# XiandaGuo/OpenStereo

Measured on AMD Instinct MI355X. Metric: stereo-pairs/s at 540x960 D=192 (GwcNet fwd), higher is better.
Workload: dtype f32 via f16x3 split-MFMA (hi/lo fp16 operands, f32 accumulate; HBM tensors f32); 1 GPU; GwcNet-gc inference, SceneFlow-shaped 540x960 padded to 544x960, D=192, G=40 + 12ch concat (BASELINE configs[1]); weights=deterministic synthetic (sharpened), random-init architecture, sub_batch_streams=3, parallelism=independent pairs x1, precision=f16x3, launch=hipGraph replay

## Files before the change

include/openstereo_amd.h:

```cpp
#ifndef OPENSTEREO_AMD_H
#define OPENSTEREO_AMD_H

#include <stddef.h>

#ifdef __cplusplus
extern "C" {
#endif

#define OSA_ABI_VERSION 16
#define OSA_META_FLOATS 128

enum { OSA_NCDHW = 0, OSA_NDHWC = 1 };
enum { OSA_ACT_NONE = 0, OSA_ACT_RELU = 1, OSA_ACT_LEAKY = 2, OSA_ACT_RELU6 = 3, OSA_ACT_SIGMOID = 4, OSA_ACT_TANH = 5 };
enum { OSA_GATE_RAW = 16 };
#define OSA_GATE_CHANNELS(n) ((int)((unsigned)(n) << 16))
enum { OSA_IN_SPLIT = 32, OSA_OUT_SPLIT = 64, OSA_RES_SPLIT = 128, OSA_REDIR_SPLIT = 256 };
enum { OSA_RES_AFTER_ACT = 512 };

int         osa_abi_version(void);
const char* osa_last_error(void);
const char* osa_target_arch(void);

int osa_build_volume_f32(const float* left_gwc, const float* right_gwc, int C, int num_groups,
                         const float* left_cat, const float* right_cat, int Cc,
                         float* vol, int layout, int vol_channels, int c_off,
                         int B, int H, int W, int maxdisp, int mask_left_concat,
                         float* vol_meta, void* stream);

int osa_build_volume_nhwc_f32(const float* left_gwc, const float* right_gwc, int C, int num_groups, int gwc_stride,
                              const float* left_cat, const float* right_cat, int Cc, int cat_stride,
                              float* vol, int vol_channels, int c_off,
                              int B, int H, int W, int maxdisp, int mask_left_concat, float* vol_meta, void* stream);
int osa_cat_fms_f32(const float* reference_fm, const float* target_fm, float* out, const int* disp_index,
                    int B, int C, int H, int W, int n_samples, void* stream);
int osa_pair_volume_f32(const float* left, const float* right, float* out,
                        int B, int C, int groups, int H, int W, int planes, int mode, void* stream);

int osa_corr_volume_f32(const float* left, const float* right, float* vol,
                        int B, int C, int H, int W, int maxdisp, void* stream);

int osa_ncdhw_to_ndhwc_f32(const float* x, float* y, int B, int C, long long S,
                           int yCs, int c_off, void* stream);
// ... 333 lines not shown

enum { OSA_IN_F16 = 32, OSA_OUT_F16 = 64, OSA_RES_F16 = 128 };
int osa_conv3d_pack_f16(const float* w_ref, float* w_packed, int Ci, int Co, int kd, int kh, int kw, void* stream);
int osa_deconv3d_pack_f16(const float* w_ref, float* w_packed, int Ci, int Co, int k, int pad, void* stream);
int osa_deconv2d_pack_f16(const float* w_ref, float* w_packed, int Ci, int Co, int k, int pad, void* stream);
int osa_conv3d_ndhwc_f16(const void* x, const float* w_packed, const float* scale, const float* shift, const void* residual, void* y,
                         int B, int Di, int Hi, int Wi, int Ci, int xCs, int Co, int yCs, int rCs, int kd, int kh, int kw, int stride,
                         int pad_d, int pad_h, int pad_w, int dil_d, int dil_h, int dil_w, const float* gate_logits, int gCs,
                         int act, float slope, void* stream);
int osa_deconv3d_ndhwc_f16(const void* x, const float* w_packed, const float* scale, const float* shift, const void* residual, void* y,
                           int B, int Di, int Hi, int Wi, int Ci, int xCs, int Co, int yCs, int rCs, int k, int pad, int opad,
                           const float* gate_logits, int gCs, int act, float slope, void* stream);
int osa_deconv2d_nhwc_f16(const void* x, const float* w_packed, const float* scale, const float* shift, const void* residual, void* y,
                          int B, int Hi, int Wi, int Ci, int xCs, int Co, int yCs, int rCs, int k, int pad, int opad,
                          const float* gate_logits, int gCs, int act, float slope, void* stream);

size_t osa_channel_sums_workspace_bytes(long long P, int C);
int osa_channel_sums(const void* dy, int dy_f16, int dy_cs, const void* x, int x_f16, int x_cs, const float* x_shift,
                     const float* dx_scale, void* dx, int dx_cs, long long P, int C,
                     float* out, float* workspace, size_t workspace_bytes, void* stream);
int osa_channel_sums_multi(const void* const* dys, int n_items, int dy_f16, int dy_cs, long long P, int C,
                           float* out, float* workspace, size_t workspace_bytes, void* stream);
int osa_channel_affine(const void* u, int u_f16, int u_cs, const void* v, int v_f16, int v_cs,
                       const float* a, const float* b, const float* c0, void* out, int out_cs,
                       long long P, int C, int relu, void* stream);

size_t osa_instnorm_workspace_floats(int B, long long HW, int C);
int osa_instnorm_nhwc_f32(const float* x, float* y, int B, long long HW, int C, int xCs, int yCs, float eps, int act, float slope,
                          float* workspace, float* y_meta, void* stream);

long long osa_conv3d_march_launches(void);

long long osa_conv3d_march_s2_launches(void);

int osa_deconv_walk(int enable);
int osa_deconv_walk_segment_planes(int planes);
long long osa_deconv3d_walk_launches(void);

int osa_conv_b_ring_mask(int mask);
long long osa_conv_b_ring_launches(void);

int osa_volume_walk_step(int step);
long long osa_volume_walk_launches(void);

int osa_build_volume_nhwc_split_eligible(const float* left_cat, const float* right_cat, const float* vol, int C, int num_groups,
                                         int gwc_stride, int Cc, int cat_stride, int vol_channels, int c_off, int W, int maxdisp);
int osa_build_volume_nhwc_split_f16x3(const float* left_gwc, const float* right_gwc, int C, int num_groups, int gwc_stride,
                                      const float* left_cat, const float* right_cat, int Cc, int cat_stride,
                                      float* vol, int vol_channels, int c_off,
                                      int B, int H, int W, int maxdisp, int mask_left_concat,
                                      const float* gwc_meta, const float* cat_meta, float* vol_meta, void* stream);

#ifdef __cplusplus
}
#endif
#endif
```

openstereo_amd/_lib.py:

```python
from __future__ import annotations

import ctypes as C
import os
import threading

_HERE = os.path.dirname(os.path.abspath(__file__))
LIB_PATH = os.environ.get("OSA_LIB_PATH") or os.path.join(_HERE, "lib", "libopenstereo_amd.so")

_lock = threading.Lock()
_lib = None

c_fp = C.c_void_p
c_i = C.c_int
c_f = C.c_float
c_st = C.c_void_p
c_ll = C.c_longlong


class F16x3Ranges(C.Structure):
    _fields_ = [("x_meta", C.c_void_p), ("residual_meta", C.c_void_p), ("redir_meta", C.c_void_p),
                ("y_meta", C.c_void_p), ("bound_coef", C.c_void_p), ("redir_bound_coef", C.c_void_p), ("weight_scale", C.c_void_p)]


c_rng = C.POINTER(F16x3Ranges)
# ... 44 lines not shown
    "osa_deconv2d_nhwc_f16x3": (c_i, [c_fp] * 6 + [c_i] * 11 + [c_fp, c_i, c_i, c_f, c_f, c_rng, c_st]),
    "osa_dwconv2d_pack_f32": (c_i, [c_fp, c_fp, c_i, c_i, c_i, c_st]),
    "osa_dwconv2d_nhwc_f32": (c_i, [c_fp] * 6 + [c_i] * 15 + [c_fp, c_st]),
    "osa_dwconv2d_nhwc_f16io": (c_i, [c_fp, c_i, c_fp, c_fp, c_fp, c_fp, c_i] + [c_i] * 11 + [c_i, c_fp, c_st]),
    "osa_gru_combine_f32": (c_i, [c_fp, c_fp, c_fp, c_fp, c_ll, c_i, c_i, c_i, c_i, c_i, c_fp, c_st]),
    "osa_gru_gates_rz_fwd": (c_i, [c_ref, c_fp, c_fp, c_ref, c_ref, c_ref, c_ref, c_ref, c_ll, c_i, c_st]),
    "osa_gru_gates_rz_bwd": (c_i, [c_ref, c_fp, c_fp, c_ref, c_ref, c_ref, c_ref, c_ref, c_ref, c_ref, c_ll, c_i, c_st]),
    "osa_gru_gates_q_fwd": (c_i, [c_ref, c_ref, c_fp, c_ref, c_ref, c_ref, c_ll, c_i, c_st]),
    "osa_gru_gates_q_bwd": (c_i, [c_ref, c_ref, c_fp, c_ref, c_ref, c_ref, c_ref, c_ref, c_ref, c_ll, c_i, c_st]),
    "osa_disp_update_f32": (c_i, [c_fp, c_fp, c_i, c_fp, c_fp, c_i, c_ll, c_fp, c_fp, c_st]),
    "osa_conv3d_pack_ex_auto": (c_i, [c_fp, c_fp, c_i, c_i, c_i, c_i, c_i, c_i, c_i, c_fp, c_fp, c_st]),
    **dict.fromkeys(("osa_deconv3d_pack_f16x3_auto", "osa_deconv2d_pack_f16x3_auto"), (c_i, [c_fp, c_fp, c_i, c_i, c_i, c_i, c_fp, c_fp, c_st])),
    "osa_cat_fms_f32": (c_i, [c_fp, c_fp, c_fp, c_fp, c_i, c_i, c_i, c_i, c_i, c_st]),
    "osa_pool2x_nhwc_f32": (c_i, [c_fp, c_fp, c_i, c_i, c_i, c_i, c_i, c_i, c_fp, c_fp, c_st]),
    "osa_resize_bilinear_nhwc_f32": (c_i, [c_fp, c_fp, c_i, c_i, c_i, c_i, c_i, c_i, c_i, c_i, c_fp, c_fp, c_st]),
    "osa_context_upsample_logits_f32": (c_i, [c_fp, c_fp, c_i, C.POINTER(c_ll), c_fp, c_i, c_i, c_i, c_i, c_f, c_st]),
    "osa_context_upsample_logits_bwd_f32": (c_i, [c_fp, c_fp, c_i, C.POINTER(c_ll), c_fp, c_fp, c_fp, C.POINTER(c_ll), c_fp, c_i, c_i, c_i, c_i, c_f, c_st]),
    "osa_context_upsample_f32": (c_i, [c_fp, c_fp, c_fp, c_i, c_i, c_i, c_i, c_i, c_f, c_st]),
    "osa_geo_rows_f32": (c_i, [c_fp, c_fp, c_i, c_i, c_i, c_i, c_i, c_i, c_st]),
    "osa_avgpool_rows_f32": (c_i, [c_fp, c_fp, c_ll, c_i, c_st]),
    **dict.fromkeys(("osa_geo_lookup_f32", "osa_geo_lookup_bwd_acc_f32", "osa_geo_lookup_bwd_f32"), (c_i, _LEVELS + [c_fp, c_fp, c_fp, c_i, c_i, c_i, c_i, c_i, c_st])),
    "osa_geo_lookup_nhwc_f32": (c_i, _LEVELS + [c_fp, c_fp, c_fp, c_i, c_i, c_i, c_i, c_i, c_i, c_st]),
    **dict.fromkeys(("osa_geo_lookup_mr_f32", "osa_geo_lookup_mr_bwd_acc_f32"), (c_i, _LEVELS + [c_fp, c_i, c_fp, c_i, c_fp, c_fp, c_fp, c_fp, c_fp, c_fp, c_i, c_i, c_i, c_i, c_i, c_st])),
    "osa_geo_lookup_mr_nhwc_f32": (c_i, _LEVELS + [c_fp, c_i, c_fp, c_i, c_fp, c_fp, c_fp, c_fp, c_fp, c_fp, c_i, c_i, c_i, c_i, c_i, c_i, c_i, c_i, c_i, c_st]),
    "osa_preprocess_pair_f32": (c_i, [c_fp, c_fp, c_i, c_i, c_i, c_i, c_i, C.POINTER(c_f), C.POINTER(c_f), c_fp, c_i, c_st]),
    "osa_instnorm_workspace_floats": (C.c_size_t, [c_i, c_ll, c_i]),
    "osa_instnorm_nhwc_f32": (c_i, [c_fp, c_fp, c_i, c_ll, c_i, c_i, c_i, c_f, c_i, c_f, c_fp, c_fp, c_st]),
    "osa_conv3d_wgrad_ws_multi": (c_i, [c_i, c_fp, c_fp, c_i, c_fp] + [c_i] * 22 + [c_fp, c_fp, c_i, c_i, c_fp, C.c_size_t, c_st]),
    "osa_channel_sums_workspace_bytes": (C.c_size_t, [c_ll, c_i]),
    "osa_channel_affine": (c_i, [c_fp, c_i, c_i, c_fp, c_i, c_i, c_fp, c_fp, c_fp, c_fp, c_i, c_ll, c_i, c_i, c_st]),
    "osa_channel_sums_multi": (c_i, [c_fp, c_i, c_i, c_i, c_ll, c_i, c_fp, c_fp, C.c_size_t, c_st]),
    "osa_channel_sums": (c_i, [c_fp, c_i, c_i, c_fp, c_i, c_i, c_fp, c_fp, c_fp, c_i, c_ll, c_i, c_fp, c_fp, C.c_size_t, c_st]),
    **dict.fromkeys(("osa_conv3d_march_launches", "osa_conv3d_march_s2_launches", "osa_deconv3d_walk_launches", "osa_conv_b_ring_launches", "osa_volume_walk_launches"), (c_ll, [])),
    **dict.fromkeys(("osa_deconv_walk", "osa_deconv_walk_segment_planes", "osa_conv_b_ring_mask", "osa_volume_walk_step"), (c_i, [c_i])),
    "osa_build_volume_nhwc_split_eligible": (c_i, [c_fp, c_fp, c_fp, c_i, c_i, c_i, c_i, c_i, c_i, c_i, c_i, c_i]),
    "osa_build_volume_nhwc_split_f16x3": (c_i, [c_fp, c_fp, c_i, c_i, c_i, c_fp, c_fp, c_i, c_i, c_fp] + [c_i] * 7 + [c_fp, c_fp, c_fp, c_st]),
    "osa_upsample_softargmin_f32": (c_i, [c_fp, c_fp, c_i, c_i, c_i, c_i, c_i, c_i, c_i, c_i, c_st]),
    **dict.fromkeys(("osa_softargmin_var_f32", "osa_softmax_softargmin_var_bwd_f32"), (c_i, [c_fp, c_fp, c_fp, c_fp, c_i, c_i, c_i, c_i, c_st])),
    "osa_softargmin_var_bwd_f32": (c_i, [c_fp, c_fp, c_fp, c_fp, c_fp, c_fp, c_i, c_i, c_i, c_i, c_st]),
    "osa_upsample_softargmin_var_bwd_ws_f32": (c_i, [c_fp, c_fp, c_fp, c_fp, c_i, c_i, c_i, c_i, c_i, c_i, c_i, c_i, c_fp, C.c_size_t, c_st]),
    "osa_mr_volume_f32": (c_i, [c_fp] * 7 + [c_i] * 12 + [c_st]),
    "osa_mr_volume_bwd_ws_f32": (c_i, [c_fp] * 3 + [c_i] + [c_fp] * 8 + [c_i] * 11 + [c_fp, C.c_size_t, c_st]),
    **dict.fromkeys(("osa_mv2_block3d_packed_floats", "osa_mv2_block2d_packed_floats"), (C.c_size_t, [c_i] * 3)),
    **dict.fromkeys(("osa_mv2_block3d_pack_f32", "osa_mv2_block2d_pack_f32"), (c_i, [c_fp] * 10 + [c_i] * 3 + [c_st])),
    "osa_mv2_block3d_f32": (c_i, [c_fp] * 3 + [c_i] * 9 + [c_st]),
    **dict.fromkeys(("osa_mv2_block2d_f32", "osa_disparity_attention_f32"), (c_i, [c_fp] * 4 + [c_i] * 9 + [c_st])),
    "osa_disparity_attention_pack_f32": (c_i, [c_fp] * 8 + [c_i] * 4 + [c_st]),
    "osa_interlaced_volume_pack_f32": (c_i, [c_fp] * 13 + [c_i] * 4 + [c_st]),
    "osa_interlaced_volume_f32": (c_i, [c_fp] * 4 + [c_i] * 8 + [c_st]),
}


class EngineError(RuntimeError):
    pass


def load():
    global _lib
    if _lib is not None:
        return _lib
    with _lock:
        if _lib is not None:
            return _lib
        if not os.path.exists(LIB_PATH):
            raise EngineError(f"{LIB_PATH} is missing: build it with `python -m openstereo_amd.build` (hipcc, gfx950). There is no CPU fallback.")
        lib = C.CDLL(LIB_PATH)
        for name, (res, args) in SIGNATURES.items():
# ... 46 lines not shown
```

openstereo_amd/csrc/conv3d.hip:

```cpp
#include "conv_kernel.h"
#include "conv_inst.h"

namespace osa {

struct KernelCfg {
    const char* name;
    int M, N;
    int TD, TH, TW, threads;
    int ks;
    int table, idx;
};

static const KernelCfg g_cfgs[] = {
#define OSA_CFG_X(RING, MT, NT, WM, WN, TH, TW)                                                                  \
    { #MT "x" #NT "_" #WM "x" #WN "_" #TH "x" #TW, WM * MT * 32, WN * NT * 32, WM * MT * 32 / (TH * TW), TH, TW, WM * WN * 64, 0, 0, -1 },
#define OSA_KS_X(MT, NT, WM, WN, TH, TW, KS)
#include "conv_cfgs.def"
#undef OSA_CFG_X
#undef OSA_KS_X
};
constexpr int N_CFGS = sizeof(g_cfgs) / sizeof(g_cfgs[0]);

static const KernelCfg g_ks_cfgs[] = {
#define OSA_CFG_X(RING, MT, NT, WM, WN, TH, TW)
// ... 132 lines not shown
    static Key cache[64]; static int used = 0;
    for (int i = 0; i < used; ++i) if (cache[i].f == (const void*)fn && cache[i].l == lds) return cache[i].n;
    int n = 0;
    if (hipOccupancyMaxActiveBlocksPerMultiprocessor(&n, (const void*)fn, threads, lds) != hipSuccess) { (void)hipGetLastError(); n = 1; }
    if (used < 64) cache[used++] = Key{(const void*)fn, lds, n};
    return n;
}

static void set_stagger(ConvArgs& a, const KernelCfg& k, void (*fn)(const ConvArgs), size_t lds, long long nwg, bool deconv, int prec) {
    a.stag_ticks = 0; a.stag_n = 0; a.stag_cus = 256;
    const int mode = exp_int("OSA_STAG", 0);
    if (!mode) return;
    const int waves = k.threads / 64;
    int slots = resident_workgroups(fn, k.threads, lds);
    { const int o = exp_int("OSA_STAG_K", 0); if (o) slots = o; }
    if (slots < 2 || nwg < (long long)2 * slots * 256) return;
    const double mfma_per_wave = (double)a.nchunks * a.T * ((double)k.M * k.N / 1024.0 / waves) * (prec == PREC_F16X3 ? 3.0 : 8.0);
    const double tap_us = mfma_per_wave * (prec == PREC_F16X3 ? 32.0 : 64.0) / 2000.0;
    const double bytes = (double)a.LD * a.LH * a.LW * 64.0 * a.nchunks + (double)k.M * (deconv ? 8 : 1) * k.N * 4.0 * (a.res || a.rx ? 2 : 1);
    const double mem_us = bytes / (4.0e6 / 256.0);
    double step_us = tap_us > mem_us ? tap_us : mem_us;
    if ((tap_us + mem_us) / slots > step_us) step_us = (tap_us + mem_us) / slots;
    { const int o = exp_int("OSA_STAG_PCT", 100); step_us *= o / 100.0; }
    { const int o = exp_int("OSA_STAG_US10", 0); if (o) step_us = o / 10.0; }
    a.stag_ticks = (int)(step_us * 100.0 + 0.5);
    a.stag_n = slots * 256; a.stag_cus = 256;
    if (exp_int("OSA_STAG_PRINT", 0)) fprintf(stderr, "[stagger] %s slots %d tap %.2f us mem %.2f us step %.2f us\n", k.name, slots, tap_us, mem_us, step_us);
}

int launch_conv_march(ConvArgs& a, hipStream_t st, const char* what);
int launch_conv_march_s2(ConvArgs& a, hipStream_t st, const char* what);
int launch_conv_deconv_walk(ConvArgs& a, hipStream_t st, const char* what);
void wgrad_set_multi_tile(int on);
void march_s2_set_waves(int w);

static int g_b_ring_mask = (1 << 1) | (1 << 2) | (1 << 3) | (1 << 4) | (1 << 13) | (1 << 29) | (1 << 27);
static long long g_b_ring_launches = 0;
static int g_b_ring_mask_value() { return g_b_ring_mask; }

static int plan_conv(ConvArgs& a, int stride, int prec, const char* what, const KernelCfg* forced, const KernelCfg*& kp) {
    int ci = forced ? 0 : pick_cfg(a, stride, prec);
    if (!forced && brick_bytes(a, g_cfgs[ci]) > 160 * 1024) {
        static const int fallback[] = {5, 15, 3, 11};
        for (int f : fallback)
            if (a.CoP % g_cfgs[f].N == 0 && brick_bytes(a, g_cfgs[f]) <= 160 * 1024) { ci = f; break; }
    }
    kp = forced ? forced : &g_cfgs[ci];
    if (!forced && (ci == 11 || ci == 14) && a.Ad == 1 && !(a.act & OSA_OUT_SPLIT)) {
        const int want = exp_int("OSA_KS", -1);
        const long long items = (prec == PREC_F32) ? 1 : a.B;
        const long long nwg = ((items * a.Ad * a.Ah * a.Aw + g_cfgs[ci].M - 1) / g_cfgs[ci].M) * (a.CoP / g_cfgs[ci].N);
        int ks = (a.nchunks % 4 == 0 && a.nchunks >= 16) ? 4 : ((a.nchunks % 2 == 0 && a.nchunks >= 8) ? 2 : 1);
        if (nwg >= 192) ks = 1;
        else if (nwg >= 96 && ks == 4) ks = 2;
        if (want >= 0) ks = (want > 1 && a.nchunks % want == 0) ? want : 1;
        const KernelCfg* split = (ks == 4) ? &g_ks_cfgs[ci == 11 ? 0 : 1] : ((ks == 2) ? &g_ks_cfgs[ci == 11 ? 2 : 3] : nullptr);
        if (split && brick_bytes(a, *split) * ks <= 160 * 1024) kp = split;
    }
    const KernelCfg& k = *kp;
    a.tilesD = cdiv(a.Ad, k.TD); a.tilesH = cdiv(a.Ah, k.TH); a.tilesW = cdiv(a.Aw, k.TW);
    (void)brick_bytes(a, k);
    OSA_REQUIRE((long long)a.LD * a.LH * a.LW < 65536, "%s: LDS brick too large", what);
    finish_geometry(a, k.TW, k.TW == 8 && a.isw == 1);
    const size_t brick = (size_t)a.LD * a.PlaneQ * sizeof(float4);
    OSA_REQUIRE(brick <= 160 * 1024, "%s: LDS brick %dx%dx%d needs %zu B (> 160 KiB)", what, a.LD, a.LH, a.LW, brick);
    return 0;
}
// ... 856 lines not shown
    OSA_REQUIRE(nblk < (1ll << 31), "conv3d_small_co: grid too large");
    dim3 grid((unsigned)nblk), block(256);
#define OSA_SC_LAUNCH1(CO, WG)                                                                              \
    do {                                                                                                    \
        if (lds > 64 * 1024)                                                                                \
            (void)hipFuncSetAttribute((const void*)conv_small_co_tiled_kernel<CO, WG>,                      \
                                      hipFuncAttributeMaxDynamicSharedMemorySize, (int)lds);                \
        hipLaunchKernelGGL((conv_small_co_tiled_kernel<CO, WG>), grid, block, lds, st, a, w_ref, bias);     \
    } while (0)
#define OSA_SC_LAUNCH(CO) do { if (packed) OSA_SC_LAUNCH1(CO, true); else OSA_SC_LAUNCH1(CO, false); } while (0)
    switch (Co) {
        case 1: OSA_SC_LAUNCH(1); break;
        case 2: OSA_SC_LAUNCH(2); break;
        case 3: OSA_SC_LAUNCH(3); break;
        default: OSA_SC_LAUNCH(4); break;
    }
#undef OSA_SC_LAUNCH
    OSA_LAUNCH_CHECK("conv3d_small_co");
    return 0;
}

#ifdef OSA_TRACE_ON
extern "C" int osa_debug_trace_read(unsigned long long* dst, size_t n_words) {
    const size_t have = (size_t)osa::TRACE_SLOTS * osa::TRACE_WAVES * osa::TRACE_EVENTS;
    if (n_words > have) n_words = have;
    if (hipDeviceSynchronize() != hipSuccess) return -1;
    if (hipMemcpyFromSymbol(dst, HIP_SYMBOL(osa::g_trace), n_words * sizeof(unsigned long long)) != hipSuccess) return -1;
    static unsigned long long zeros[osa::TRACE_SLOTS * osa::TRACE_WAVES * osa::TRACE_EVENTS];
    if (hipMemcpyToSymbol(HIP_SYMBOL(osa::g_trace), zeros, sizeof(zeros)) != hipSuccess) return -1;
    return (int)n_words;
}
#endif

extern "C" int osa_conv_b_ring_mask(int mask) { const int prev = osa::g_b_ring_mask; osa::g_b_ring_mask = mask; osa::march_s2_set_waves(((mask >> 28) & 1) ? 4 : 8); osa::wgrad_set_multi_tile((mask >> 27) & 1); return prev; }
extern "C" long long osa_conv_b_ring_launches(void) { return osa::g_b_ring_launches; }
```

openstereo_amd/csrc/conv_march.hip:

```cpp
#include "conv_march.h"
#include "conv_march_s2.h"
#include "conv_deconv_walk.h"

namespace osa {

static long long g_march_launches = 0;
long long march_launches() { return g_march_launches; }

struct MarchCfg { int nwv, tw, th; size_t lds; void (*fn[2][2])(const ConvArgs, int, int); };
#define OSA_MARCH_CFG(NWV, TW) { NWV, TW, MarchGeo<NWV, TW>::TH, MarchGeo<NWV, TW>::lds_bytes(),                      \
                                 { { conv_march_kernel<NWV, TW, 0, 0>, conv_march_kernel<NWV, TW, 0, 1> },            \
                                   { conv_march_kernel<NWV, TW, 1, 0>, conv_march_kernel<NWV, TW, 1, 1> } } }
static const MarchCfg g_march_cfgs[] = {
    OSA_MARCH_CFG(4, 16),
    OSA_MARCH_CFG(4, 32),
};

int launch_conv_march(ConvArgs& a, hipStream_t st, const char* what) {
    if (!exp_int("OSA_MARCH", 1)) return 0;
    if (a.T != 27 || a.Co != 32 || a.CoP != 32 || a.Di < 3 || a.gate || a.rx) return 0;
    if (a.Ci % 16 != 0) return 0;
    const int actk = a.act & 15;
    if (actk > OSA_ACT_LEAKY || (a.act & (OSA_GATE_RAW | OSA_RES_AFTER_ACT)) || ((unsigned)a.act >> 16)) return 0;
    if ((a.yCs & 3) || ((size_t)a.y & 15) || (a.res && ((a.rCs & 3) || ((size_t)a.res & 15)))) return 0;
// ... 28 lines not shown
    const long long cols = (long long)a.B * a.tilesH * a.tilesW;
    int per_cu = (int)((160 * 1024) / g.lds);
    if (per_cu > 8 / g.nwv) per_cu = 8 / g.nwv;
    const long long slots = (long long)per_cu * 256;
    int nseg = 1;
    {
        double best = 1e30;
        for (int n = 1; n <= 16 && n * 2 <= a.Di; ++n) {
            const int ds = cdiv(a.Di, n), ns = cdiv(a.Di, ds);
            if (ns != n) continue;
            const double cost = (double)((cols * ns + slots - 1) / slots) * (ds + (ns > 1 ? 2.0 : 0.0));
            if (cost < best - 1e-9) { best = cost; nseg = ns; }
        }
        const int o = exp_int("OSA_MARCH_NSEG", 0);
        if (o > 0 && o * 2 <= a.Di) nseg = o;
    }
    const int dseg = cdiv(a.Di, nseg);
    nseg = cdiv(a.Di, dseg);
    OSA_REQUIRE(cols * nseg < (1ll << 31), "%s: grid too large", what);
    void (*fn)(const ConvArgs, int, int) = g.fn[(a.act & OSA_OUT_SPLIT) ? 1 : 0][(a.act & OSA_IN_SPLIT) ? 1 : 0];
    static bool attr_set[2][2][2];
    bool& done = attr_set[gi][(a.act & OSA_OUT_SPLIT) ? 1 : 0][(a.act & OSA_IN_SPLIT) ? 1 : 0];
    if (!done && g.lds > 64 * 1024) { (void)hipFuncSetAttribute((const void*)fn, hipFuncAttributeMaxDynamicSharedMemorySize, (int)g.lds); }
    done = true;
    hipLaunchKernelGGL(fn, dim3((unsigned)(cols * nseg)), dim3(g.nwv * 64), g.lds, st, a, dseg, nseg);
    OSA_LAUNCH_CHECK(what);
    ++g_march_launches;
    return 1;
}

static long long g_march_s2_launches = 0;
long long march_s2_launches() { return g_march_s2_launches; }

static int g_march_s2_waves = 8;
template <int NWV>
static int launch_conv_march_s2_t(ConvArgs& a, hipStream_t st, const char* what) {
    using G = MarchS2Geo<NWV>;
    a.tilesD = 1; a.tilesH = cdiv(a.Ho, G::TH); a.tilesW = cdiv(a.Wo, G::TW);
    a.dbg = exp_int("OSA_DBG", 0);
    const long long cols = (long long)a.B * a.tilesH * a.tilesW;
    const long long slots = 256 * (NWV == 8 ? 1 : 2);
    int nseg = 1;
    {
        double best = 1e30;
        for (int n = 1; n <= a.Do; ++n) {
            const int os = cdiv(a.Do, n), ns = cdiv(a.Do, os);
            if (ns != n) continue;
            const double cost = (double)((cols * ns + slots - 1) / slots) * (2.0 * os + (ns > 1 ? 1.0 : 0.0) + 0.5);
            if (cost < best - 1e-9) { best = cost; nseg = ns; }
        }
        const int o = exp_int("OSA_MARCH_NSEG", 0);
        if (o > 0 && o <= a.Do) nseg = o;
    }
    const int oseg = cdiv(a.Do, nseg);
    nseg = cdiv(a.Do, oseg);
    OSA_REQUIRE(cols * nseg < (1ll << 31), "%s: grid too large", what);
    static bool attr_set = false;
    if (!attr_set) { (void)hipFuncSetAttribute((const void*)conv_march_s2_kernel<NWV>, hipFuncAttributeMaxDynamicSharedMemorySize, (int)G::lds_bytes()); attr_set = true; }
    hipLaunchKernelGGL(conv_march_s2_kernel<NWV>, dim3((unsigned)(cols * nseg)), dim3(NWV * 64), G::lds_bytes(), st, a, oseg, nseg);
    OSA_LAUNCH_CHECK(what);
    return 1;
}

void march_s2_set_waves(int w) { g_march_s2_waves = (w == 4) ? 4 : 8; }

int launch_conv_march_s2(ConvArgs& a, hipStream_t st, const char* what) {
    if (a.T != 27 || a.Co != 64 || a.CoP != 64 || a.Di < 2 || a.gate || a.rx || a.res) return 0;
    if (a.Ci % 16 != 0 || a.xCs % 16 != 0) return 0;
    if (!(a.act & OSA_IN_SPLIT) || !(a.act & OSA_OUT_SPLIT)) return 0;
    const int actk = a.act & 15;
    if (actk > OSA_ACT_LEAKY || (a.act & (OSA_GATE_RAW | OSA_RES_AFTER_ACT)) || ((unsigned)a.act >> 16)) return 0;
    if ((a.yCs % 16) || ((size_t)a.y & 15) || ((size_t)a.x & 15)) return 0;
    if ((long long)a.Do * a.Ho * a.Wo * a.yCs >= (1ll << 31)) return 0;
    if ((long long)a.Hi * a.Wi * a.xCs >= (1ll << 29)) return 0;
    const int r = g_march_s2_waves == 8 ? launch_conv_march_s2_t<8>(a, st, what) : launch_conv_march_s2_t<4>(a, st, what);
    if (r == 1) ++g_march_s2_launches;
    return r;
}

static long long g_deconv_walk_launches = 0;
long long deconv_walk_launches() { return g_deconv_walk_launches; }

static int g_deconv_walk = 2;
int deconv_walk_set(int enable) { const int prev = g_deconv_walk; g_deconv_walk = enable & 3; return prev; }
static int g_deconv_walk_planes = 0;
int deconv_walk_planes_set(int planes) { const int prev = g_deconv_walk_planes; g_deconv_walk_planes = planes > 0 ? planes : 0; return prev; }

template <int WN, int RCH>
static int launch_conv_deconv_walk_t(ConvArgs& a, hipStream_t st, const char* what) {
    using G = DeconvWalkGeo<WN>;
    a.tilesD = 1; a.tilesH = cdiv(a.Hi, G::TH); a.tilesW = cdiv(a.Wi, G::TW);
    for (int t = 0, c = 0; t < a.T; ++t) {
        while (t >= a.cls_end[c]) ++c;
        const int kd = ((c >> 2) & 1) ? (a.td[t] == 1 ? 0 : 2) : 1;
        const int kh = ((c >> 1) & 1) ? (a.th[t] == 1 ? 0 : 2) : 1;
        const int kw = (c & 1) ? (a.tw[t] == 1 ? 0 : 2) : 1;
        a.toff[kd * 9 + kh * 3 + kw] = t;
    }
    const long long cols = (long long)a.B * a.tilesH * a.tilesW;
    const long long slots = 2 * 256;
    int nseg = 1;
    {
        double best = 1e30;
        for (int n = 1; n <= a.Do; ++n) {
            const int os = cdiv(a.Do, n), ns = cdiv(a.Do, os);
            if (ns != n) continue;
            const double cost = (double)((cols * ns + slots - 1) / slots) * (1.5 * os + 0.5);
            if (cost < best - 1e-9) { best = cost; nseg = ns; }
        }
    }
    int oseg = cdiv(a.Do, nseg);
    if (g_deconv_walk_planes > 0) oseg = g_deconv_walk_planes < a.Do ? g_deconv_walk_planes : a.Do;
    nseg = cdiv(a.Do, oseg);
    OSA_REQUIRE(cols * nseg < (1ll << 31), "%s: grid too large", what);
    OSA_REQUIRE(hipFuncSetAttribute((const void*)conv_deconv_walk_kernel<WN, RCH>, hipFuncAttributeMaxDynamicSharedMemorySize, (int)G::lds_bytes()) == hipSuccess,
                "%s: %d bytes of LDS per workgroup refused", what, (int)G::lds_bytes());
    hipLaunchKernelGGL((conv_deconv_walk_kernel<WN, RCH>), dim3((unsigned)(cols * nseg)), dim3(G::NWV * 64), G::lds_bytes(), st, a, oseg, nseg);
    OSA_LAUNCH_CHECK(what);
    return 1;
}

int launch_conv_deconv_walk(ConvArgs& a, hipStream_t st, const char* what) {
    if (a.T != 27 || a.Do != 2 * a.Di || a.Ho != 2 * a.Hi || a.Wo != 2 * a.Wi) return 0;
    if (!a.rx || a.res || a.gate) return 0;
    const int cls = (a.Co == 32 && a.rCi == 32) ? 0 : ((a.Co == 64 && a.rCi == 64) ? 1 : -1);
    if (cls < 0 || a.CoP != a.Co || !((g_deconv_walk >> cls) & 1)) return 0;
    if (!(a.act & OSA_IN_SPLIT) || !(a.act & OSA_OUT_SPLIT) || !(a.act & OSA_REDIR_SPLIT)) return 0;
    const int actk = a.act & 15;
    if (actk > OSA_ACT_LEAKY || (a.act & (OSA_GATE_RAW | OSA_RES_AFTER_ACT)) || ((unsigned)a.act >> 16)) return 0;
    if (a.Ci % 16 != 0 || a.xCs % 16 != 0 || a.yCs % 16 != 0 || a.rxCs % 16 != 0) return 0;
    if (((size_t)a.x & 15) || ((size_t)a.y & 15) || ((size_t)a.rx & 15)) return 0;
    if ((long long)a.Do * a.Ho * a.Wo * (a.yCs > a.rxCs ? a.yCs : a.rxCs) >= (1ll << 31)) return 0;
    if ((long long)a.Hi * a.Wi * a.xCs >= (1ll << 29)) return 0;
    const int r = cls == 0 ? launch_conv_deconv_walk_t<1, 2>(a, st, what) : launch_conv_deconv_walk_t<2, 4>(a, st, what);
    if (r == 1) ++g_deconv_walk_launches;
    return r;
}

}

extern "C" long long osa_conv3d_march_launches(void) { return osa::march_launches(); }
extern "C" long long osa_conv3d_march_s2_launches(void) { return osa::march_s2_launches(); }
extern "C" long long osa_deconv3d_walk_launches(void) { return osa::deconv_walk_launches(); }
extern "C" int osa_deconv_walk(int enable) { return osa::deconv_walk_set(enable); }
extern "C" int osa_deconv_walk_segment_planes(int planes) { return osa::deconv_walk_planes_set(planes); }
```

openstereo_amd/csrc/conv_march_s2.h:

```cpp
#pragma once
#include "conv_kernel.h"

namespace osa {

template <int NWV_>
struct MarchS2Geo {
    static constexpr int NWV = NWV_, TW = 32, TH = NWV_ / 2;
    static constexpr int LH = 2 * TH + 1, LW = 2 * TW + 1, NEV = TW + 1;
    static constexpr int NVOX = LH * LW;
    static constexpr int NPI = (NVOX * 4 + 63) / 64;
    static constexpr int PLANEQ = NPI * 64;
    static constexpr int NP = (NPI + NWV - 1) / NWV;
    static constexpr int BRING = 3, BSTEPQ = 12 * 64;
    static constexpr int NIB = NWV == 8 ? 2 : 3;
    static constexpr size_t lds_bytes() { return (size_t)2 * PLANEQ * 16 + (size_t)BRING * BSTEPQ * 16; }
    static_assert((size_t)NWV * 32 * 36 * 4 <= (size_t)PLANEQ * 16, "epilogue tiles must fit into one plane buffer");
};

template <int N>
__device__ __forceinline__ void wait_vmcnt_c() {
    static_assert(N >= 0 && N <= 15, "vmcnt immediate");
    if constexpr (N == 0) asm volatile("s_waitcnt vmcnt(0)" ::: "memory");
    else if constexpr (N == 1) asm volatile("s_waitcnt vmcnt(1)" ::: "memory");
    else if constexpr (N == 2) asm volatile("s_waitcnt vmcnt(2)" ::: "memory");
    else if constexpr (N == 3) asm volatile("s_waitcnt vmcnt(3)" ::: "memory");
    else if constexpr (N == 4) asm volatile("s_waitcnt vmcnt(4)" ::: "memory");
    else if constexpr (N == 5) asm volatile("s_waitcnt vmcnt(5)" ::: "memory");
    else if constexpr (N == 6) asm volatile("s_waitcnt vmcnt(6)" ::: "memory");
    else if constexpr (N == 7) asm volatile("s_waitcnt vmcnt(7)" ::: "memory");
    else if constexpr (N == 8) asm volatile("s_waitcnt vmcnt(8)" ::: "memory");
    else asm volatile("s_waitcnt vmcnt(9)" ::: "memory");
}

template <int NWV_>
__global__ __launch_bounds__(NWV_ * 64, 2) void conv_march_s2_kernel(const ConvArgs p, const int oseg, const int nseg) {
    using G = MarchS2Geo<NWV_>;
    constexpr int PLANEQ = G::PLANEQ, NP = G::NP, NPI = G::NPI, NWV = G::NWV, NIB = G::NIB, TH = G::TH, TW = G::TW, LW = G::LW, NEV = G::NEV;
    extern __shared__ __attribute__((aligned(16))) float4 smem[];
    float4* const bring = smem + 2 * PLANEQ;

    const int tid = threadIdx.x, lane = tid & 63;
    const int wv = __builtin_amdgcn_readfirstlane(tid >> 6);
    const int wm = wv & (TH - 1), wn = wv / TH;
    const int col = lane & 31, hh = lane >> 5;

    unsigned bid = xcd_remap(blockIdx.x, gridDim.x);
    const int twi = bid % p.tilesW; bid /= p.tilesW;
    const int thi = bid % p.tilesH; bid /= p.tilesH;
    const int seg = bid % nseg;
    const int b = (int)(bid / nseg);
    const int o0 = seg * oseg, o1 = (o0 + oseg < p.Do) ? o0 + oseg : p.Do;
    const int a0h = thi * TH, a0w = twi * TW;
    const int g0h = 2 * a0h - 1, g0w = 2 * a0w - 1;

    float s_in = 1.f, s_out = 1.f;
    if (p.in_meta) s_in = p.in_meta[1];
    if (p.coef && p.in_meta) s_out = pow2_scale((p.coef[0] * amax_read(p.in_meta) + p.coef[1]) * 1.0625f);
    if (p.out_meta && blockIdx.x == 0 && tid == 0) p.out_meta[1] = s_out;
    const float osc = (p.wscale_dev ? p.wscale_dev[1] : p.oscale) * (1.0f / s_in);
    float am = 0.f;
    unsigned amax_seen = 0u;
    if (p.out_meta) amax_seen = amax_peek(p.out_meta);

    f32x16 acc0, acc1;
#pragma unroll
    for (int r = 0; r < 16; ++r) { acc0[r] = 0.f; acc1[r] = 0.f; }

    const int CoP = p.CoP;
    const int nch = p.nchunks;
    const int c8 = (lane & 3) * 8, vs2 = lane >> 2;
    const int actk = p.act & 15;
    const float act_ns = (actk == OSA_ACT_NONE) ? 1.f : ((actk == OSA_ACT_LEAKY) ? p.slope : 0.f);
    const bool act_relu = actk == OSA_ACT_RELU;
    float* const yb = p.y + (size_t)b * p.Do * p.Ho * p.Wo * p.yCs;

    auto dma = [&](const char* src, const unsigned lds_byte) { lds_dma16(src, lds_byte); };
    const unsigned smem_lds = (unsigned)(size_t)(__attribute__((address_space(3))) char*)smem;
    const unsigned bring_lds = smem_lds + 2u * PLANEQ * 16u;
    const char* const zsrc = reinterpret_cast<const char*>(g_lds_dma_zeros);

    unsigned boff[NIB], bdst[NIB];
#pragma unroll
    for (int i = 0; i < NIB; ++i) {
        const int f = NWV == 8 ? (i == 0 ? wv : 8 + (wv & 3)) : wv * 3 + i;
        const int kw = f >> 2, hl = (f >> 1) & 1, n = f & 1;
        boff[i] = (unsigned)((kw * 4 * CoP + hl * 2 * CoP + hh * CoP + n * 32 + col) * 16);
        bdst[i] = (unsigned)(f * 64 * 16);
    }
    auto dma_b = [&](const int slot, const int ch, const int kh, const int kd) {
        const char* base = reinterpret_cast<const char*>(p.w) + (size_t)((ch * 27 + kd * 9 + kh * 3) * 4 * CoP) * 16;
#pragma unroll
        for (int i = 0; i < NIB; ++i) dma(base + boff[i], bring_lds + (unsigned)(slot * G::BSTEPQ * 16) + bdst[i]);
    };

    unsigned poff[NP];
    unsigned pvalid = 0u;
#pragma unroll
    for (int i = 0; i < NP; ++i) {
        int n = i * NWV + wv;
        n = n < NPI ? n : NPI - 1;
        const int j = n * 64 + lane;
        const int v = j >> 2, q = (j & 3) ^ ((v >> 2) & 3);
        const int lh = v / LW, r = v - lh * LW;
        const int lw = (r < NEV) ? 2 * r : 2 * (r - NEV) + 1;
        const int gh = g0h + lh, gw = g0w + lw;
        const bool ok = v < G::NVOX && (unsigned)gh < (unsigned)p.Hi && (unsigned)gw < (unsigned)p.Wi;
        poff[i] = ok ? (unsigned)(((gh * p.Wi + gw) * p.xCs + q * 4) * 4) : 0u;
        pvalid |= ok ? (1u << i) : 0u;
    }
    const size_t plane_bytes = (size_t)p.Hi * p.Wi * p.xCs * 4;
    const char* const xb = reinterpret_cast<const char*>(p.x) + (size_t)b * p.Di * plane_bytes;
    auto dma_plane = [&](const int buf, const int pd, const int c) {
        const char* base = xb + (size_t)(pd < 0 ? 0 : pd) * plane_bytes + (size_t)c * (CC * 4);
#pragma unroll
        for (int i = 0; i < NP; ++i) {
            int n = i * NWV + wv;
            n = n < NPI ? n : NPI - 1;
            const bool ok = ((pvalid >> i) & 1u) && pd >= 0;
            dma(ok ? base + poff[i] : zsrc, smem_lds + (unsigned)((buf * PLANEQ + n * 64) * 16));
        }
    };

    auto epilogue = [&](const int od, float* const tb) {
        float4 sc[2], sh[2];
#pragma unroll
        for (int h2 = 0; h2 < 2; ++h2) {
            const int co = wn * 32 + c8 + 4 * h2;
            sc[h2] = make_float4(osc, osc, osc, osc); sh[h2] = make_float4(0.f, 0.f, 0.f, 0.f);
            if (p.scale) {
                sc[h2] = *reinterpret_cast<const float4*>(p.scale + co); sh[h2] = *reinterpret_cast<const float4*>(p.shift + co);
                sc[h2].x *= osc; sc[h2].y *= osc; sc[h2].z *= osc; sc[h2].w *= osc;
            }
        }
#pragma unroll
        for (int r = 0; r < 16; ++r) tb[((r & 3) + 8 * (r >> 2) + 4 * hh) * 36 + col] = acc0[r];
        const int oh = a0h + wm;
        const int soff = wn * 32 + (c8 >> 4) * 16 + ((c8 & 15) >> 3) * 4;
#pragma unroll
        for (int k = 0; k < 2; ++k) {
            const int ow = a0w + vs2 + 16 * k;
            const bool ok = oh < p.Ho && ow < p.Wo;
            const int vox = (od * p.Ho + oh) * p.Wo + ow;
            uint2 hq[2], lq[2];
#pragma unroll
            for (int h2 = 0; h2 < 2; ++h2) {
                const float4 a = *reinterpret_cast<const float4*>(tb + (vs2 + 16 * k) * 36 + c8 + 4 * h2);
                float o[4] = {fmaf(a.x, sc[h2].x, sh[h2].x), fmaf(a.y, sc[h2].y, sh[h2].y), fmaf(a.z, sc[h2].z, sh[h2].z), fmaf(a.w, sc[h2].w, sh[h2].w)};
#pragma unroll
                for (int e = 0; e < 4; ++e) o[e] = (o[e] < 0.f) ? (act_relu ? 0.f : o[e] * act_ns) : o[e];
                if (ok) am = fmaxf(am, fmaxf(fmaxf(fabsf(o[0]), fabsf(o[1])), fmaxf(fabsf(o[2]), fabsf(o[3]))));
                split_f16(make_float4(o[0] * s_out, o[1] * s_out, o[2] * s_out, o[3] * s_out), hq[h2], lq[h2]);
            }
            if (ok) {
                float* ys = yb + (size_t)vox * p.yCs + soff;
                store16(ys, make_uint4(hq[0].x, hq[0].y, hq[1].x, hq[1].y));
                store16(ys + 8, make_uint4(lq[0].x, lq[0].y, lq[1].x, lq[1].y));
            }
        }
    };

    auto taps = [&](f32x16& acc, const int cur, const int slot, const int kh) {
        const int vrow = (2 * wm + kh) * LW + col;
        float4 A[3][2], Bf[3][2];
#pragma unroll
        for (int kw = 0; kw < 3; ++kw) {
            const int v = vrow + (kw == 1 ? NEV : (kw >> 1));
            const int qs = hh ^ ((v >> 2) & 3);
            A[kw][0] = smem[cur * PLANEQ + 4 * v + qs];
            A[kw][1] = smem[cur * PLANEQ + 4 * v + (qs ^ 2)];
            Bf[kw][0] = bring[slot * G::BSTEPQ + ((kw * 2 + 0) * 2 + wn) * 64 + lane];
            Bf[kw][1] = bring[slot * G::BSTEPQ + ((kw * 2 + 1) * 2 + wn) * 64 + lane];
        }
#pragma unroll
        for (int kw = 0; kw < 3; ++kw)
#pragma unroll
            for (int term = 0; term < 3; ++term) {
                const f16x8 a = __builtin_bit_cast(f16x8, A[kw][term == 1 ? 1 : 0]);
                const f16x8 w = __builtin_bit_cast(f16x8, Bf[kw][term == 0 ? 1 : 0]);
                acc = __builtin_amdgcn_mfma_f32_32x32x16_f16(a, w, acc, 0, 0, 0);
            }
    };

    const int pf = (2 * o0 - 1 > 0) ? 2 * o0 - 1 : 0;
    const int pl = (2 * o1 - 1 < p.Di - 1) ? 2 * o1 - 1 : p.Di - 1;
    auto steps_of = [&](const int pd) { const int od = pd >> 1; return (pd & 1) ? ((od >= o0 ? 3 : 0) + (od + 1 < o1 ? 3 : 0)) : 3; };
    auto kd_of = [&](const int pd, const int k) { return (pd & 1) ? ((k < 3 && (pd >> 1) >= o0) ? 2 : 0) : 1; };
    int lpd = pf, lc = 0, lk = 0;
    bool ldone = false;
    auto issue_b = [&](const int slot) {
        dma_b(slot, lc, lk >= 3 ? lk - 3 : lk, kd_of(lpd, lk));
        if (!ldone) {
            if (++lk == steps_of(lpd)) {
                lk = 0;
                if (++lc == nch) { lc = 0; ++lpd; }
                if (lpd > pl) { ldone = true; lpd = pl; lc = nch - 1; lk = steps_of(pl) - 1; }
            }
        }
    };

    dma_plane(0, pf, 0);
    issue_b(0); issue_b(1);
    wait_vmcnt_c<0>();

    int slot = 0;
    int q = 0;
    for (int pd = pf; pd <= pl; ++pd) {
        const bool odd = pd & 1;
        const int od = pd >> 1;
        const bool do0 = !odd || od >= o0;
        const int ns = steps_of(pd);
        for (int c = 0; c < nch; ++c, ++q) {
            const int cur = q & 1;
            int npd = pd, nc = c + 1;
            if (nc == nch) { nc = 0; ++npd; }
            if (npd > pl) npd = -1;
            for (int k = 0; k < ns; ++k) {
                __syncthreads();
                issue_b(slot >= 1 ? slot - 1 : 2);
                if (k == 0) dma_plane(cur ^ 1, npd, nc);
                const int kh = k >= 3 ? k - 3 : k;
                if (odd && !(k < 3 && do0)) taps(acc1, cur, slot, kh);
                else taps(acc0, cur, slot, kh);
                if (k <= 1) wait_vmcnt_c<NIB + NP>(); else wait_vmcnt_c<NIB>();
                slot = slot == 2 ? 0 : slot + 1;
            }
            if (c + 1 == nch) {
                const bool fin = odd || pd == p.Di - 1;
                if (fin && od >= o0 && od < o1) {
                    __syncthreads();
                    epilogue(od, reinterpret_cast<float*>(smem + cur * PLANEQ) + wv * (32 * 36));
                }
                if (odd) {
                    acc0 = acc1;
#pragma unroll
                    for (int r = 0; r < 16; ++r) acc1[r] = 0.f;
                }
            }
        }
    }
    wait_vmcnt_c<0>();
    if (p.out_meta) {
        __syncthreads();
        publish_amax(p.out_meta, am, amax_seen, reinterpret_cast<float*>(smem));
    }
}

}
```

Measured before the change: 194.0 stereo-pairs/s.

## Stage full 9-tap weight slab per kd in stride-2 march conv, double-buffered

Replaces the 3-slot per-kh weight ring in the stride-2 march conv3d kernel with a double-buffered slab holding all 9 (kh,kw) taps for one kd. Each barrier interval now runs 27 MFMAs with software-pipelined A/B LDS loads instead of 9, so there are fewer __syncthreads and DMA issue points. The 4-wave variant and its mask toggle are dropped, and the kernel is fixed at 8 waves with occupancy 1 because LDS use is larger. An override for planes per segment is added, and the segment cost model is retuned. The risks are lower occupancy, more LDS, and a full vmcnt(0) wait on most steps.

```diff
diff --git a/include/openstereo_amd.h b/include/openstereo_amd.h
--- a/include/openstereo_amd.h
+++ b/include/openstereo_amd.h
@@ -7,7 +7,7 @@
 extern "C" {
 #endif
 
-#define OSA_ABI_VERSION 16
+#define OSA_ABI_VERSION 17
 #define OSA_META_FLOATS 128
 
 enum { OSA_NCDHW = 0, OSA_NDHWC = 1 };
@@ -407,6 +407,7 @@
 long long osa_conv3d_march_launches(void);
 
 long long osa_conv3d_march_s2_launches(void);
+int osa_conv_march_s2_segment_planes(int planes);
 
 int osa_deconv_walk(int enable);
 int osa_deconv_walk_segment_planes(int planes);
diff --git a/openstereo_amd/_lib.py b/openstereo_amd/_lib.py
--- a/openstereo_amd/_lib.py
+++ b/openstereo_amd/_lib.py
@@ -100,7 +100,7 @@
     "osa_channel_sums_multi": (c_i, [c_fp, c_i, c_i, c_i, c_ll, c_i, c_fp, c_fp, C.c_size_t, c_st]),
     "osa_channel_sums": (c_i, [c_fp, c_i, c_i, c_fp, c_i, c_i, c_fp, c_fp, c_fp, c_i, c_ll, c_i, c_fp, c_fp, C.c_size_t, c_st]),
     **dict.fromkeys(("osa_conv3d_march_launches", "osa_conv3d_march_s2_launches", "osa_deconv3d_walk_launches", "osa_conv_b_ring_launches", "osa_volume_walk_launches"), (c_ll, [])),
-    **dict.fromkeys(("osa_deconv_walk", "osa_deconv_walk_segment_planes", "osa_conv_b_ring_mask", "osa_volume_walk_step"), (c_i, [c_i])),
+    **dict.fromkeys(("osa_deconv_walk", "osa_deconv_walk_segment_planes", "osa_conv_march_s2_segment_planes", "osa_conv_b_ring_mask", "osa_volume_walk_step"), (c_i, [c_i])),
     "osa_build_volume_nhwc_split_eligible": (c_i, [c_fp, c_fp, c_fp, c_i, c_i, c_i, c_i, c_i, c_i, c_i, c_i, c_i]),
     "osa_build_volume_nhwc_split_f16x3": (c_i, [c_fp, c_fp, c_i, c_i, c_i, c_fp, c_fp, c_i, c_i, c_fp] + [c_i] * 7 + [c_fp, c_fp, c_fp, c_st]),
     "osa_upsample_softargmin_f32": (c_i, [c_fp, c_fp, c_i, c_i, c_i, c_i, c_i, c_i, c_i, c_i, c_st]),
diff --git a/openstereo_amd/csrc/conv3d.hip b/openstereo_amd/csrc/conv3d.hip
--- a/openstereo_amd/csrc/conv3d.hip
+++ b/openstereo_amd/csrc/conv3d.hip
@@ -188,7 +188,6 @@
 int launch_conv_march_s2(ConvArgs& a, hipStream_t st, const char* what);
 int launch_conv_deconv_walk(ConvArgs& a, hipStream_t st, const char* what);
 void wgrad_set_multi_tile(int on);
-void march_s2_set_waves(int w);
 
 static int g_b_ring_mask = (1 << 1) | (1 << 2) | (1 << 3) | (1 << 4) | (1 << 13) | (1 << 29) | (1 << 27);
 static long long g_b_ring_launches = 0;
@@ -1111,5 +1110,5 @@
 }
 #endif
 
-extern "C" int osa_conv_b_ring_mask(int mask) { const int prev = osa::g_b_ring_mask; osa::g_b_ring_mask = mask; osa::march_s2_set_waves(((mask >> 28) & 1) ? 4 : 8); osa::wgrad_set_multi_tile((mask >> 27) & 1); return prev; }
+extern "C" int osa_conv_b_ring_mask(int mask) { const int prev = osa::g_b_ring_mask; osa::g_b_ring_mask = mask; osa::wgrad_set_multi_tile((mask >> 27) & 1); return prev; }
 extern "C" long long osa_conv_b_ring_launches(void) { return osa::g_b_ring_launches; }
diff --git a/openstereo_amd/csrc/conv_march.hip b/openstereo_amd/csrc/conv_march.hip
--- a/openstereo_amd/csrc/conv_march.hip
+++ b/openstereo_amd/csrc/conv_march.hip
@@ -84,37 +84,8 @@
 static long long g_march_s2_launches = 0;
 long long march_s2_launches() { return g_march_s2_launches; }
 
-static int g_march_s2_waves = 8;
-template <int NWV>
-static int launch_conv_march_s2_t(ConvArgs& a, hipStream_t st, const char* what) {
-    using G = MarchS2Geo<NWV>;
-    a.tilesD = 1; a.tilesH = cdiv(a.Ho, G::TH); a.tilesW = cdiv(a.Wo, G::TW);
-    a.dbg = exp_int("OSA_DBG", 0);
-    const long long cols = (long long)a.B * a.tilesH * a.tilesW;
-    const long long slots = 256 * (NWV == 8 ? 1 : 2);
-    int nseg = 1;
-    {
-        double best = 1e30;
-        for (int n = 1; n <= a.Do; ++n) {
-            const int os = cdiv(a.Do, n), ns = cdiv(a.Do, os);
-            if (ns != n) continue;
-            const double cost = (double)((cols * ns + slots - 1) / slots) * (2.0 * os + (ns > 1 ? 1.0 : 0.0) + 0.5);
-            if (cost < best - 1e-9) { best = cost; nseg = ns; }
-        }
-        const int o = exp_int("OSA_MARCH_NSEG", 0);
-        if (o > 0 && o <= a.Do) nseg = o;
-    }
-    const int oseg = cdiv(a.Do, nseg);
-    nseg = cdiv(a.Do, oseg);
-    OSA_REQUIRE(cols * nseg < (1ll << 31), "%s: grid too large", what);
-    static bool attr_set = false;
-    if (!attr_set) { (void)hipFuncSetAttribute((const void*)conv_march_s2_kernel<NWV>, hipFuncAttributeMaxDynamicSharedMemorySize, (int)G::lds_bytes()); attr_set = true; }
-    hipLaunchKernelGGL(conv_march_s2_kernel<NWV>, dim3((unsigned)(cols * nseg)), dim3(NWV * 64), G::lds_bytes(), st, a, oseg, nseg);
-    OSA_LAUNCH_CHECK(what);
-    return 1;
-}
-
-void march_s2_set_waves(int w) { g_march_s2_waves = (w == 4) ? 4 : 8; }
+static int g_march_s2_planes = 0;
+int march_s2_planes_set(int planes) { const int prev = g_march_s2_planes; g_march_s2_planes = planes > 0 ? planes : 0; return prev; }
 
 int launch_conv_march_s2(ConvArgs& a, hipStream_t st, const char* what) {
     if (a.T != 27 || a.Co != 64 || a.CoP != 64 || a.Di < 2 || a.gate || a.rx || a.res) return 0;
@@ -125,9 +96,34 @@
     if ((a.yCs % 16) || ((size_t)a.y & 15) || ((size_t)a.x & 15)) return 0;
     if ((long long)a.Do * a.Ho * a.Wo * a.yCs >= (1ll << 31)) return 0;
     if ((long long)a.Hi * a.Wi * a.xCs >= (1ll << 29)) return 0;
-    const int r = g_march_s2_waves == 8 ? launch_conv_march_s2_t<8>(a, st, what) : launch_conv_march_s2_t<4>(a, st, what);
-    if (r == 1) ++g_march_s2_launches;
-    return r;
+    using G = MarchS2Geo;
+    a.tilesD = 1; a.tilesH = cdiv(a.Ho, G::TH); a.tilesW = cdiv(a.Wo, G::TW);
+    const long long cols = (long long)a.B * a.tilesH * a.tilesW;
+    const long long slots = 256;
+    int nseg = 1;
+    {
+        double best = 1e30;
+        for (int n = 1; n <= a.Do; ++n) {
+            const int os = cdiv(a.Do, n), ns = cdiv(a.Do, os);
+            if (ns != n) continue;
+            const double cost = (double)((cols * ns + slots - 1) / slots) * (3.0 * os + (ns > 1 ? 1.0 : 0.0) + 1.5);
+            if (cost < best - 1e-9) { best = cost; nseg = ns; }
+        }
+    }
+    int oseg = cdiv(a.Do, nseg);
+    if (g_march_s2_planes > 0) oseg = g_march_s2_planes < a.Do ? g_march_s2_planes : a.Do;
+    nseg = cdiv(a.Do, oseg);
+    OSA_REQUIRE(cols * nseg < (1ll << 31), "%s: grid too large", what);
+    static bool attr_set = false;
+    if (!attr_set) {
+        OSA_REQUIRE(hipFuncSetAttribute((const void*)conv_march_s2_kernel, hipFuncAttributeMaxDynamicSharedMemorySize, (int)G::lds_bytes()) == hipSuccess,
+                    "%s: %d bytes of LDS per workgroup refused", what, (int)G::lds_bytes());
+        attr_set = true;
+    }
+    hipLaunchKernelGGL(conv_march_s2_kernel, dim3((unsigned)(cols * nseg)), dim3(G::NWV * 64), G::lds_bytes(), st, a, oseg, nseg);
+    OSA_LAUNCH_CHECK(what);
+    ++g_march_s2_launches;
+    return 1;
 }
 
 static long long g_deconv_walk_launches = 0;
@@ -193,6 +189,7 @@
 
 extern "C" long long osa_conv3d_march_launches(void) { return osa::march_launches(); }
 extern "C" long long osa_conv3d_march_s2_launches(void) { return osa::march_s2_launches(); }
+extern "C" int osa_conv_march_s2_segment_planes(int planes) { return osa::march_s2_planes_set(planes); }
 extern "C" long long osa_deconv3d_walk_launches(void) { return osa::deconv_walk_launches(); }
 extern "C" int osa_deconv_walk(int enable) { return osa::deconv_walk_set(enable); }
 extern "C" int osa_deconv_walk_segment_planes(int planes) { return osa::deconv_walk_planes_set(planes); }
diff --git a/openstereo_amd/csrc/conv_march_s2.h b/openstereo_amd/csrc/conv_march_s2.h
--- a/openstereo_amd/csrc/conv_march_s2.h
+++ b/openstereo_amd/csrc/conv_march_s2.h
@@ -3,19 +3,20 @@
 
 namespace osa {
 
-template <int NWV_>
 struct MarchS2Geo {
-    static constexpr int NWV = NWV_, TW = 32, TH = NWV_ / 2;
+    static constexpr int NWV = 8, TW = 32, TH = 4;
     static constexpr int LH = 2 * TH + 1, LW = 2 * TW + 1, NEV = TW + 1;
     static constexpr int NVOX = LH * LW;
     static constexpr int NPI = (NVOX * 4 + 63) / 64;
     static constexpr int PLANEQ = NPI * 64;
     static constexpr int NP = (NPI + NWV - 1) / NWV;
-    static constexpr int BRING = 3, BSTEPQ = 12 * 64;
-    static constexpr int NIB = NWV == 8 ? 2 : 3;
-    static constexpr size_t lds_bytes() { return (size_t)2 * PLANEQ * 16 + (size_t)BRING * BSTEPQ * 16; }
+    static constexpr int NBI = 9 * 4;
+    static constexpr int BSLABQ = NBI * 64;
+    static constexpr int NIB = (NBI + NWV - 1) / NWV;
+    static constexpr size_t lds_bytes() { return (size_t)2 * PLANEQ * 16 + (size_t)2 * BSLABQ * 16; }
     static_assert((size_t)NWV * 32 * 36 * 4 <= (size_t)PLANEQ * 16, "epilogue tiles must fit into one plane buffer");
 };
+static_assert(MarchS2Geo::lds_bytes() <= 160 * 1024, "one workgroup must fit into the LDS of a CU");
 
 template <int N>
 __device__ __forceinline__ void wait_vmcnt_c() {
@@ -32,12 +33,11 @@
     else asm volatile("s_waitcnt vmcnt(9)" ::: "memory");
 }
 
-template <int NWV_>
-__global__ __launch_bounds__(NWV_ * 64, 2) void conv_march_s2_kernel(const ConvArgs p, const int oseg, const int nseg) {
-    using G = MarchS2Geo<NWV_>;
-    constexpr int PLANEQ = G::PLANEQ, NP = G::NP, NPI = G::NPI, NWV = G::NWV, NIB = G::NIB, TH = G::TH, TW = G::TW, LW = G::LW, NEV = G::NEV;
+__global__ __launch_bounds__(MarchS2Geo::NWV * 64, 1) void conv_march_s2_kernel(const ConvArgs p, const int oseg, const int nseg) {
+    using G = MarchS2Geo;
+    constexpr int PLANEQ = G::PLANEQ, NP = G::NP, NPI = G::NPI, NWV = G::NWV, NIB = G::NIB, NBI = G::NBI, BSLABQ = G::BSLABQ, TH = G::TH, TW = G::TW, LW = G::LW, NEV = G::NEV;
     extern __shared__ __attribute__((aligned(16))) float4 smem[];
-    float4* const bring = smem + 2 * PLANEQ;
+    float4* const bslab = smem + 2 * PLANEQ;
 
     const int tid = threadIdx.x, lane = tid & 63;
     const int wv = __builtin_amdgcn_readfirstlane(tid >> 6);
@@ -76,21 +76,17 @@
 
     auto dma = [&](const char* src, const unsigned lds_byte) { lds_dma16(src, lds_byte); };
     const unsigned smem_lds = (unsigned)(size_t)(__attribute__((address_space(3))) char*)smem;
-    const unsigned bring_lds = smem_lds + 2u * PLANEQ * 16u;
+    const unsigned bslab_lds = smem_lds + 2u * PLANEQ * 16u;
     const char* const zsrc = reinterpret_cast<const char*>(g_lds_dma_zeros);
 
-    unsigned boff[NIB], bdst[NIB];
-#pragma unroll
-    for (int i = 0; i < NIB; ++i) {
-        const int f = NWV == 8 ? (i == 0 ? wv : 8 + (wv & 3)) : wv * 3 + i;
-        const int kw = f >> 2, hl = (f >> 1) & 1, n = f & 1;
-        boff[i] = (unsigned)((kw * 4 * CoP + hl * 2 * CoP + hh * CoP + n * 32 + col) * 16);
-        bdst[i] = (unsigned)(f * 64 * 16);
-    }
-    auto dma_b = [&](const int slot, const int ch, const int kh, const int kd) {
-        const char* base = reinterpret_cast<const char*>(p.w) + (size_t)((ch * 27 + kd * 9 + kh * 3) * 4 * CoP) * 16;
-#pragma unroll
-        for (int i = 0; i < NIB; ++i) dma(base + boff[i], bring_lds + (unsigned)(slot * G::BSTEPQ * 16) + bdst[i]);
+    auto dma_b = [&](const int buf, const int ch, const int kd) {
+        const char* base = reinterpret_cast<const char*>(p.w) + (size_t)((ch * 27 + kd * 9) * 4 * CoP) * 16 + lane * 16;
+#pragma unroll
+        for (int i = 0; i < NIB; ++i) {
+            int n = i * NWV + wv;
+            n = n < NBI ? n : NBI - 1;
+            dma(base + n * 1024, bslab_lds + (unsigned)((buf * BSLABQ + n * 64) * 16));
+        }
     };
 
     unsigned poff[NP];
@@ -111,13 +107,12 @@
     const size_t plane_bytes = (size_t)p.Hi * p.Wi * p.xCs * 4;
     const char* const xb = reinterpret_cast<const char*>(p.x) + (size_t)b * p.Di * plane_bytes;
     auto dma_plane = [&](const int buf, const int pd, const int c) {
-        const char* base = xb + (size_t)(pd < 0 ? 0 : pd) * plane_bytes + (size_t)c * (CC * 4);
+        const char* base = xb + (size_t)pd * plane_bytes + (size_t)c * (CC * 4);
 #pragma unroll
         for (int i = 0; i < NP; ++i) {
             int n = i * NWV + wv;
             n = n < NPI ? n : NPI - 1;
-            const bool ok = ((pvalid >> i) & 1u) && pd >= 0;
-            dma(ok ? base + poff[i] : zsrc, smem_lds + (unsigned)((buf * PLANEQ + n * 64) * 16));
+            dma(((pvalid >> i) & 1u) ? base + poff[i] : zsrc, smem_lds + (unsigned)((buf * PLANEQ + n * 64) * 16));
         }
     };
 
@@ -159,70 +154,73 @@
         }
     };
 
-    auto taps = [&](f32x16& acc, const int cur, const int slot, const int kh) {
-        const int vrow = (2 * wm + kh) * LW + col;
-        float4 A[3][2], Bf[3][2];
-#pragma unroll
-        for (int kw = 0; kw < 3; ++kw) {
-            const int v = vrow + (kw == 1 ? NEV : (kw >> 1));
-            const int qs = hh ^ ((v >> 2) & 3);
-            A[kw][0] = smem[cur * PLANEQ + 4 * v + qs];
-            A[kw][1] = smem[cur * PLANEQ + 4 * v + (qs ^ 2)];
-            Bf[kw][0] = bring[slot * G::BSTEPQ + ((kw * 2 + 0) * 2 + wn) * 64 + lane];
-            Bf[kw][1] = bring[slot * G::BSTEPQ + ((kw * 2 + 1) * 2 + wn) * 64 + lane];
-        }
-#pragma unroll
-        for (int kw = 0; kw < 3; ++kw)
+    int aq[9];
+#pragma unroll
+    for (int t = 0; t < 9; ++t) {
+        const int kh = t / 3, kw = t % 3;
+        const int v = (2 * wm + kh) * LW + col + (kw == 1 ? NEV : (kw >> 1));
+        aq[t] = 4 * v + (hh ^ ((v >> 2) & 3));
+    }
+    const int bq = hh * 64 + wn * 32 + col;
+    auto taps = [&](f32x16& acc, const int cur, const int wb) {
+        const float4* const pa = smem + cur * PLANEQ;
+        const float4* const pb = bslab + wb * BSLABQ + bq;
+        float4 A[2][2], Bf[2][2];
+        A[0][0] = pa[aq[0]]; A[0][1] = pa[aq[0] ^ 2];
+        Bf[0][0] = pb[0]; Bf[0][1] = pb[2 * 64];
+#pragma unroll
+        for (int t = 0; t < 9; ++t) {
+            const int s = t & 1;
+            if (t + 1 < 9) {
+                A[s ^ 1][0] = pa[aq[t + 1]]; A[s ^ 1][1] = pa[aq[t + 1] ^ 2];
+                Bf[s ^ 1][0] = pb[((t + 1) * 4 + 0) * 64]; Bf[s ^ 1][1] = pb[((t + 1) * 4 + 2) * 64];
+            }
 #pragma unroll
             for (int term = 0; term < 3; ++term) {
-                const f16x8 a = __builtin_bit_cast(f16x8, A[kw][term == 1 ? 1 : 0]);
-                const f16x8 w = __builtin_bit_cast(f16x8, Bf[kw][term == 0 ? 1 : 0]);
+                const f16x8 a = __builtin_bit_cast(f16x8, A[s][term == 1 ? 1 : 0]);
+                const f16x8 w = __builtin_bit_cast(f16x8, Bf[s][term == 0 ? 1 : 0]);
                 acc = __builtin_amdgcn_mfma_f32_32x32x16_f16(a, w, acc, 0, 0, 0);
             }
+        }
     };
 
     const int pf = (2 * o0 - 1 > 0) ? 2 * o0 - 1 : 0;
     const int pl = (2 * o1 - 1 < p.Di - 1) ? 2 * o1 - 1 : p.Di - 1;
-    auto steps_of = [&](const int pd) { const int od = pd >> 1; return (pd & 1) ? ((od >= o0 ? 3 : 0) + (od + 1 < o1 ? 3 : 0)) : 3; };
-    auto kd_of = [&](const int pd, const int k) { return (pd & 1) ? ((k < 3 && (pd >> 1) >= o0) ? 2 : 0) : 1; };
-    int lpd = pf, lc = 0, lk = 0;
-    bool ldone = false;
-    auto issue_b = [&](const int slot) {
-        dma_b(slot, lc, lk >= 3 ? lk - 3 : lk, kd_of(lpd, lk));
-        if (!ldone) {
-            if (++lk == steps_of(lpd)) {
-                lk = 0;
-                if (++lc == nch) { lc = 0; ++lpd; }
-                if (lpd > pl) { ldone = true; lpd = pl; lc = nch - 1; lk = steps_of(pl) - 1; }
-            }
+    auto subs_of = [&](const int pd) { const int od = pd >> 1; return (pd & 1) ? ((od >= o0 ? 1 : 0) + (od + 1 < o1 ? 1 : 0)) : 1; };
+    auto kd_of = [&](const int pd, const int j) { return (pd & 1) ? ((j == 0 && (pd >> 1) >= o0) ? 2 : 0) : 1; };
+    int lpd = pf, lc = 0, lj = 0;
+    auto issue_b = [&](const int buf) {
+        dma_b(buf, lc, kd_of(lpd, lj));
+        if (++lj == subs_of(lpd)) {
+            lj = 0;
+            if (++lc == nch) { lc = 0; ++lpd; }
         }
     };
 
     dma_plane(0, pf, 0);
-    issue_b(0); issue_b(1);
+    issue_b(0);
     wait_vmcnt_c<0>();
 
-    int slot = 0;
+    int wb = 0;
     int q = 0;
     for (int pd = pf; pd <= pl; ++pd) {
         const bool odd = pd & 1;
         const int od = pd >> 1;
         const bool do0 = !odd || od >= o0;
-        const int ns = steps_of(pd);
+        const int ns = subs_of(pd);
         for (int c = 0; c < nch; ++c, ++q) {
             const int cur = q & 1;
             int npd = pd, nc = c + 1;
             if (nc == nch) { nc = 0; ++npd; }
-            if (npd > pl) npd = -1;
-            for (int k = 0; k < ns; ++k) {
+            for (int j = 0; j < ns; ++j) {
                 __syncthreads();
-                issue_b(slot >= 1 ? slot - 1 : 2);
-                if (k == 0) dma_plane(cur ^ 1, npd, nc);
-                const int kh = k >= 3 ? k - 3 : k;
-                if (odd && !(k < 3 && do0)) taps(acc1, cur, slot, kh);
-                else taps(acc0, cur, slot, kh);
-                if (k <= 1) wait_vmcnt_c<NIB + NP>(); else wait_vmcnt_c<NIB>();
-                slot = slot == 2 ? 0 : slot + 1;
+                if (lpd <= pl) issue_b(wb ^ 1);
+                const bool stage = j == 0 && npd <= pl;
+                if (stage) dma_plane(cur ^ 1, npd, nc);
+                if (odd && !(j == 0 && do0)) taps(acc1, cur, wb);
+                else taps(acc0, cur, wb);
+                if (stage && j + 1 < ns) wait_vmcnt_c<NP>(); else wait_vmcnt_c<0>();
+                wb ^= 1;
             }
             if (c + 1 == nch) {
                 const bool fin = odd || pd == p.Di - 1;
@@ -238,7 +236,6 @@
             }
         }
     }
-    wait_vmcnt_c<0>();
     if (p.out_meta) {
         __syncthreads();
         publish_amax(p.out_meta, am, amax_seen, reinterpret_cast<float*>(smem));
```

Result: faster. 196.0 stereo-pairs/s (median of 6 runs) (+1.0%).
